# christang/alignment-algos

Hardware: AMD Instinct MI355X
Metric: GCUPS (DP cell updates/s) at 1/2/4/8 MI355X; bit-exact score vs ref (higher is better)
Workload: dtype int32

## Files before the change

### alignment-algos_amd/csrc/aln_device.h

```cpp
#pragma once
#include "aln_internal.h"

namespace aln {

__device__ __forceinline__ float clip0(float s, bool local) {
  return local ? ((0.f < s) ? s : 0.f) : s;
}
__device__ __forceinline__ float fminr(float a, float b) { return (b < a) ? b : a; }

struct EvalDev {
  int Q, T;
  int model, align_type;
  float gi, ge;
  const float* tgi;
  const float* tge;
  const float* tcn;
  const float* deltab;
  const int64_t* deltab_off;
  const float* instab;
  int sim_kind;
  const uint8_t* qc; const uint8_t* tc;
  const float* tablef;
  const float* S; int ld;
};

__device__ __forceinline__ float dev_deletion(const EvalDev& e, int t1, int t2) {
  const bool free_end = (e.align_type == ALN_LOCAL || e.align_type == ALN_SEMI_LOCAL || e.align_type == ALN_LOCAL_GLOBAL);
  if (e.model == ALN_GAP_AFFINE_CONST) {
    int len = t2 - t1 - 1;
    if (len < 1) return 0.f;
    if (free_end && (t1 == 0 || t2 == e.T - 1)) return 0.f;
    return e.gi + e.ge * (float)(len - 1);
  } else if (e.model == ALN_GAP_DEL_TABLE_INS_TPOS || e.model == ALN_GAP_TABLES) {
    return e.deltab[(size_t)t1 * e.T + t2];
  } else {
    int dist = t2 - t1;
    if (dist < 2) return 0.f;
    float gi = fminr(e.tgi[t1], e.tgi[t2]);
    float ge = fminr(e.tge[t1], e.tge[t2]);
    if (free_end && (t1 == 0 || t2 == e.T - 1)) return 0.f;
    return gi + ge * (float)(dist - 2);
  }
}
__device__ __forceinline__ float dev_insertion(const EvalDev& e, int q1, int q2, int t1, int t2) {
  const bool free_end = (e.align_type == ALN_LOCAL || e.align_type == ALN_SEMI_LOCAL || e.align_type == ALN_GLOBAL_LOCAL);
  if (e.model == ALN_GAP_AFFINE_CONST) {
    int len = q2 - q1 - 1;
    if (len < 1) return 0.f;
    if (free_end && (q1 == 0 || q2 == e.Q - 1)) return 0.f;
    return e.gi + e.ge * (float)(len - 1);
  } else if (e.model == ALN_GAP_TABLES) {
    const size_t QT = (size_t)e.Q * e.T;
    if (q1 == 0) return e.instab[QT + (size_t)t1 * e.Q + q2];
    if (q2 == e.Q - 1) return e.instab[2 * QT + (size_t)t1 * e.Q + q1];
    return e.instab[(size_t)t1 * e.Q + (q2 - q1)];
  } else if (e.model == ALN_GAP_DEL_TABLE_INS_TPOS) {
    int dist = q2 - q1;
    if (dist < 2) return 0.f;
    float gp = e.tgi[t1] + e.tge[t1] * (float)(dist - 2);
    gp = gp + e.tcn[t1];
    if (free_end && (q1 == 0 || q2 == e.Q - 1)) return 0.f;
    return gp;
  } else {
    int dist = q2 - q1;
    if (dist < 2) return 0.f;
    float gi = fminr(e.tgi[t1], e.tgi[t2]);
    float ge = fminr(e.tge[t1], e.tge[t2]);
    if (free_end && (q1 == 0 || q2 == e.Q - 1)) return 0.f;
    return gi + ge * (float)(dist - 2);
  }
}
__device__ __forceinline__ void bind_table_model(EvalDev& e, const EvalDev& proto, const PairDesc& pd) {
  e.tcn = proto.tcn ? proto.tcn + pd.t_off : nullptr;
  e.deltab = proto.deltab ? proto.deltab + proto.deltab_off[pd.t_seq] : nullptr;
  e.instab = proto.instab ? proto.instab + pd.ins_off : nullptr;
}
__device__ __forceinline__ float dev_sim(const EvalDev& e, int i, int j) {
  if (e.sim_kind == ALN_SIM_SUBMATRIX) {
    if (i <= 0 || j <= 0 || i >= e.Q - 1 || j >= e.T - 1) return 0.f;
    return e.tablef[(int)e.qc[i] * 32 + (int)e.tc[j]];
  }
  return e.S[(size_t)i * e.ld + j] + 0.0f;
}

struct Frame {
  int q0, q1, t0, t1, rev;
  __device__ __forceinline__ int nQ() const { return q1 - q0; }
  __device__ __forceinline__ int nT() const { return t1 - t0; }
  __device__ __forceinline__ int rq(int a) const { return rev ? q1 - a : q0 + a; }
  __device__ __forceinline__ int rt(int b) const { return rev ? t1 - b : t0 + b; }
};

__device__ __forceinline__ float frame_del(const EvalDev& e, const Frame& f, int blo, int bhi) {
  int x = f.rt(blo), y = f.rt(bhi);
  return dev_deletion(e, x < y ? x : y, x < y ? y : x);
}
__device__ __forceinline__ float frame_ins(const EvalDev& e, const Frame& f, int alo, int ahi, int blo, int bhi) {
  int x = f.rq(alo), y = f.rq(ahi), u = f.rt(blo), v = f.rt(bhi);
  return dev_insertion(e, x < y ? x : y, x < y ? y : x, u < v ? u : v, u < v ? v : u);
}

__device__ __forceinline__ uint32_t pack_ptr(int pq, int pt) { return ((uint32_t)pq << 16) | ((uint32_t)pt & 0xFFFFu); }

__host__ __device__ __forceinline__ void decode_ptr(uint32_t w, int mode, int i, int j, int& pq, int& pt) {
  if (w == 0xFFFFFFFFu) { pq = -1; pt = -1; return; }
  if (mode == 0) { pq = (int)(w >> 16); pt = (int)(w & 0xFFFFu); if (pq == 0xFFFF) pq = -1; if (pt == 0xFFFF) pt = -1; return; }
  const int tb = mode == 2 ? 12 : 11, tmax = (1 << tb) - 1;
  const int prio = (int)((w >> tb) & 3u), k = tmax - (int)(w & (uint32_t)tmax);
  if (prio == 3) { pq = i - 1; pt = j - 1; }
  else if (prio == 2) { pq = i - 1; pt = k; }
  else { pq = k; pt = j - 1; }
}
__host__ __device__ __forceinline__ uint32_t load_ptr_word(const uint32_t* Pbase, int64_t plane_off, int ld, int i, int j, int mode) {
  const size_t e = (size_t)plane_off + (size_t)i * ld + j;
  if (mode == 0) return Pbase[e];
  const uint16_t w = reinterpret_cast<const uint16_t*>(Pbase)[e];
  return w == 0xFFFFu ? 0xFFFFFFFFu : (uint32_t)w;
}
__host__ __device__ __forceinline__ void store_ptr_word(uint32_t* Pbase, int64_t plane_off, int ld, int i, int j, int mode, uint32_t w) {
  const size_t e = (size_t)plane_off + (size_t)i * ld + j;
  if (mode == 0) Pbase[e] = w;
  else reinterpret_cast<uint16_t*>(Pbase)[e] = (uint16_t)(w & 0xFFFFu);
}
__host__ __device__ __forceinline__ float load_score(const float* Hbase, int64_t plane_off, int ld, int i, int j, int hmode) {
  const size_t e = (size_t)plane_off + (size_t)i * ld + j;
  if (hmode == 0) return Hbase[e];
  return (float)reinterpret_cast<const uint16_t*>(Hbase)[e];
}
__host__ __device__ __forceinline__ float flag_score(uint32_t w) { return (w != 0xFFFFFFFFu && (w & 0x8000u)) ? 1.f : 0.f; }
__host__ __device__ __forceinline__ void store_score(float* Hbase, int64_t plane_off, int ld, int i, int j, int hmode, float v) {
  const size_t e = (size_t)plane_off + (size_t)i * ld + j;
  if (hmode == 0) Hbase[e] = v;
  else reinterpret_cast<uint16_t*>(Hbase)[e] = (uint16_t)(int)v;
}
__host__ __device__ __forceinline__ uint32_t encode_ptr(int mode, int i, int j, int pq, int pt) {
  if (mode == 0) return ((uint32_t)pq << 16) | ((uint32_t)pt & 0xFFFFu);
  const int tb = mode == 2 ? 12 : 11, tmax = (1 << tb) - 1;
  if (pq == i - 1 && pt == j - 1) return 3u << tb;
  if (pq == i - 1) return (2u << tb) | (uint32_t)(tmax - pt);
  return (1u << tb) | (uint32_t)(tmax - pq);
}

}
```

### alignment-algos_amd/csrc/dp_affine_tag.hip

```cpp
#include <algorithm>
#include <cmath>
#include <cstdio>
#include <cstdlib>

#include "aln_internal.h"
#include "dp_tag_common.h"

namespace aln {

__device__ __forceinline__ void setprio_dyn(int p) {
  switch (p & 3) {
    case 0: __builtin_amdgcn_s_setprio(0); break;
    case 1: __builtin_amdgcn_s_setprio(1); break;
    case 2: __builtin_amdgcn_s_setprio(2); break;
    default: __builtin_amdgcn_s_setprio(3); break;
  }
}

template <int NW, int R, bool LOCAL, bool H16, int KBT, int X, bool SEGQ, int TB, int OCC, bool LEAN = false>
__global__ __launch_bounds__(64 * NW) __attribute__((amdgpu_waves_per_eu(R * X == 16 ? OCC : 1, R * X == 16 ? OCC : 8))) void dp_affine_tag_kernel(
    const PairDesc* __restrict__ pairs, const uint8_t* __restrict__ qcodes, const uint8_t* __restrict__ tcodes,
    const int32_t* __restrict__ table32, float* __restrict__ Hbase, uint32_t* __restrict__ Pbase,
    PairResult* __restrict__ res, TagParams prm) {
  typedef TagBits<TB> tag;
  constexpr int TAGMAX = tag::TAGMAX, P_MATCH = tag::P_MATCH, P_DEL = tag::P_DEL, P_INS = tag::P_INS;
  constexpr int ZKEY = tag::ZKEY, ORIGIN_DEL = tag::ORIGIN_DEL, ORIGIN_INS = tag::ORIGIN_INS;
  constexpr int KB = (KBT == 16) ? 16 : TB + 2;
  constexpr int LOW = (1 << KB) - 1;
  constexpr int NEGK = (KBT == 16) ? -(1 << 29) : tag::NEGK;
  static_assert(KBT == 13 || (KBT == 16 && LOCAL && H16), "the 16-bit key layout needs non-negative 15-bit scores");
  static_assert(TB == 11 || TB == 12, "11 or 12 tag bits");
  static_assert(X == 4 || X == 8, "a lane owns 4 or 8 consecutive columns of each group");
  static_assert(!LEAN || (NW == 2 && R == 2 && X == 8 && LOCAL && H16 && KBT == 16 && TB == 11 && !SEGQ), "one lean shape: the 16-bit key layout, whole pairs");
  constexpr int GW = 64 * X;
  __shared__ int tab[32 * 32];
  __shared__ uint8_t qcs[1 << TB];
  constexpr int RING = 16;
  __shared__ __attribute__((aligned(16))) int xch[RING][NW][4];
  __shared__ int red[NW][2];

  __shared__ int s_item;
  int pair_id = blockIdx.x, seg = 0;
  if constexpr (SEGQ) {
    if (threadIdx.x == 0) {
      const int t = __hip_atomic_fetch_add(&prm.queue[0], 1, __ATOMIC_RELAXED, __HIP_MEMORY_SCOPE_AGENT) + 1;
      int item;
      if (t < prm.n_pairs) item = t * 8;
      else {
        const int* slot = &prm.queue[16 + (t - prm.n_pairs)];
        long spins = 0;
        while ((item = __hip_atomic_load(slot, __ATOMIC_RELAXED, __HIP_MEMORY_SCOPE_AGENT)) < 0) {
          __builtin_amdgcn_s_sleep(32);
          if (++spins > (1L << 24)) {
            __hip_atomic_store(&prm.queue[2], 1, __ATOMIC_RELAXED, __HIP_MEMORY_SCOPE_AGENT);
            item = -2;
            break;
          }
        }
        __builtin_amdgcn_fence(__ATOMIC_ACQUIRE, "agent");
        asm volatile("s_waitcnt vmcnt(0)" ::: "memory");
      }
      s_item = item;
    }
    __syncthreads();
    const int item = s_item;
    if (item < 0) return;
    pair_id = item >> 3; seg = item & 7;
  }
  const PairDesc pd = pairs[pair_id];
  const int Q = pd.Q, T = pd.T, ld = pd.ld;
  const int n_seg = SEGQ ? seg_count(Q, prm.ksegs) : 1;
  const int i_begin = seg_bound(Q, seg, n_seg), i_end = seg_bound(Q, seg + 1, n_seg);
  const int lane = threadIdx.x & 63;
  const int w = __builtin_amdgcn_readfirstlane(threadIdx.x >> 6);
  const int W0 = w * GW * R;
  const int cb = W0 + X * lane;
  const int gi = prm.gi, ge = prm.ge;
  float* __restrict__ H = Hbase + pd.plane_off;
  uint16_t* __restrict__ P = reinterpret_cast<uint16_t*>(Pbase) + pd.plane_off;
  const uint8_t* __restrict__ qc = qcodes + pd.q_off;
  const uint8_t* __restrict__ tc = tcodes + pd.t_off;

  for (int k = threadIdx.x; k < 32 * 32; k += 64 * NW) tab[k] = table32[k] * (1 << KB);
  for (int k = threadIdx.x; k < Q; k += 64 * NW) qcs[k] = qc[k];
  __syncthreads();

  int inm[R][X];
  int code4[R][X];
  int GK[R][X];
  int EK[R][X];
  bool inrange[R];
#pragma unroll
  for (int r = 0; r < R; ++r) {
    inrange[r] = (cb + GW * r) < ld;
#pragma unroll
    for (int x = 0; x < X; ++x) {
      const int c = cb + GW * r + x;
      int code = kCodeTail;
      if (c < T) code = tc[c];
      code4[r][x] = code * 4;
      inm[r][x] = ((unsigned)(c - 1) < (unsigned)(T - 2)) ? -1 : 0;
      GK[r][x] = (((ge * c) * (1 << KB)) | P_DEL | (TAGMAX - (c & TAGMAX))) - P_MATCH;
      EK[r][x] = (ge * c + gi - ge) * (1 << KB);
    }
  }
  const int CB = W0 + GW * R;
  int codeB4 = kCodeTail * 4;
  if (NW > 1 && CB < T) codeB4 = tc[CB] * 4;

  int dk[R][X];
  int gmx[R][X];
  int cvk[R];
  int ak[R][X];
  uint32_t pf[R][X];
#pragma unroll
  for (int r = 0; r < R; ++r) {
    cvk[r] = NEGK;
#pragma unroll
    for (int x = 0; x < X; ++x) { dk[r][x] = P_MATCH; gmx[r][x] = NEGK; pf[r][x] = kNullPtr; }
  }
  int lmax = P_MATCH; uint32_t lpos = 0;
  const int lag = (NW > 1) ? prm.lag : 0;

  typedef unsigned int u32x2 __attribute__((ext_vector_type(2)));
  typedef unsigned int u32x4 __attribute__((ext_vector_type(4)));
  uint16_t* const H16p = reinterpret_cast<uint16_t*>(Hbase) + pd.plane_off;
  const int vo16 = cb * 2;
  auto store_words = [&](const uint32_t (&wd)[X / 2], __amdgpu_buffer_rsrc_t rs, int off) {
    if constexpr (X == 4) { const u32x2 v = {wd[0], wd[1]}; __builtin_amdgcn_raw_buffer_store_b64(v, rs, off, 0, 0); }
    else { const u32x4 v = {wd[0], wd[1], wd[2], wd[3]}; __builtin_amdgcn_raw_buffer_store_b128(v, rs, off, 0, 0); }
  };
  int own_r = -1;
  uint32_t flag_bits = 0x80008000u, sel_high = 0x07060302u;
  if constexpr (LEAN) {
    asm volatile("" : "+v"(flag_bits), "+v"(sel_high));
    const int tchunk = (T - 2) / X;
    own_r = ((tchunk & 63) == lane) ? (tchunk >> 6) - w * R : -1;
  }
  auto store_row = [&](int i, bool border = false) {
    const size_t ro = (size_t)i * ld + cb;
    const __amdgpu_buffer_rsrc_t rsP = __builtin_amdgcn_make_buffer_rsrc(P + (size_t)i * ld, 0, ld * 2, 0x00020000);
    const __amdgpu_buffer_rsrc_t rsH = __builtin_amdgcn_make_buffer_rsrc(H16p + (size_t)i * ld, 0, ld * 2, 0x00020000);
    if constexpr (LEAN) {
      const bool whole = i == Q - 2;
      asm volatile("" : "+v"(own_r));
#pragma unroll
      for (int r = 0; r < R; ++r) {
        uint32_t pw[X / 2], hw[X / 2];
#pragma unroll
        for (int x = 0; x < X; x += 2) {
          pw[x / 2] = __builtin_amdgcn_perm(pf[r][x + 1], pf[r][x], 0x05040100u);
          hw[x / 2] = __builtin_amdgcn_perm((uint32_t)dk[r][x + 1], (uint32_t)dk[r][x], sel_high);
          pw[x / 2] |= (hw[x / 2] + 0x7FFF7FFFu) & flag_bits;
        }
        if (whole || (!border && own_r == r)) store_words(hw, rsH, vo16 + 2 * GW * r);
        store_words(pw, rsP, vo16 + 2 * GW * r);
      }
      return;
    }
#pragma unroll
    for (int r = 0; r < R; ++r) {
      uint32_t pw[X / 2], hw[X / 2];
#pragma unroll
      for (int x = 0; x < X; x += 2) pw[x / 2] = __builtin_amdgcn_perm(pf[r][x + 1], pf[r][x], 0x05040100u);
      if (H16) {
#pragma unroll
        for (int x = 0; x < X; x += 2)
          hw[x / 2] = (KBT == 16) ? __builtin_amdgcn_perm((uint32_t)dk[r][x + 1], (uint32_t)dk[r][x], 0x07060302u)
                                  : (((uint32_t)dk[r][x] >> KB) | (((uint32_t)dk[r][x + 1] >> KB) << 16));
        store_words(hw, rsH, vo16 + 2 * GW * r);
      } else if (inrange[r]) {
        const float sc = 1.0f / (float)(1 << KB);
#pragma unroll
        for (int x = 0; x < X; x += 4)
          *reinterpret_cast<float4*>(H + ro + GW * r + x) =
              make_float4((float)(dk[r][x] - P_MATCH) * sc, (float)(dk[r][x + 1] - P_MATCH) * sc, (float)(dk[r][x + 2] - P_MATCH) * sc,
                          (float)(dk[r][x + 3] - P_MATCH) * sc);
      }
      store_words(pw, rsP, vo16 + 2 * GW * r);
    }
  };
  auto tab_at = [&](int qrow, int c4) -> int {
    return *reinterpret_cast<const int*>(reinterpret_cast<const char*>(tab) + qrow + c4);
  };

  auto finish_row = [&](int i, int dB, uint32_t pB, bool sync, const int4 (&xin)[NW > 1 ? NW - 1 : 1]) {
    int sk = NEGK;
    int ik[R];
#pragma unroll
    for (int r = 0; r < R; ++r) {
#pragma unroll
      for (int x = 0; x < X; ++x) ak[r][x] = dk[r][x] + GK[r][x];
      int a0 = ak[r][0];
      if (r == 0) a0 = (lane == 0) ? NEGK : a0;
      int t0 = max(a0, ak[r][1]), t1 = max(ak[r][2], ak[r][3]);
      if constexpr (X == 8) { t0 = max(max(t0, ak[r][4]), ak[r][5]); t1 = max(max(t1, ak[r][6]), ak[r][7]); }
      ik[r] = max(t0, t1);
    }
    wave_incl_max_keys<R>(ik);
#pragma unroll
    for (int r = 0; r < R; ++r) {
      const int ek = tdpp<0x138>(NEGK, ik[r]);
      cvk[r] = max(sk, ek);
      sk = max(sk, __builtin_amdgcn_readlane(ik[r], 63));
    }
    if (NW > 1) {
      const int slot = i & (RING - 1);
      if (lane == 63) { xch[slot][w][0] = sk; xch[slot][w][1] = dB; xch[slot][w][2] = (int)pB; }
      if (sync) asm volatile("s_waitcnt lgkmcnt(0)\n\ts_barrier" ::: "memory");
      if (w > 0) {
        int fk = NEGK;
        int d0 = P_MATCH; uint32_t p0 = kNullPtr;
#pragma unroll
        for (int v = 0; v < NW - 1; ++v) {
          if (v < w) {
            const int4 t = sync ? *reinterpret_cast<const int4*>(&xch[slot][v][0]) : xin[v];
            fk = max(fk, t.x);
            if (v < w - 1) {
              const int Cn = (v + 1) * GW * R;
              fk = max(fk, t.y + ((((ge * Cn) * (1 << KB)) | P_DEL | (TAGMAX - Cn)) - P_MATCH));
            } else {
              d0 = t.y; p0 = (uint32_t)t.z;
            }
          }
        }
        if (lane == 0) { dk[0][0] = d0; pf[0][0] = p0; ak[0][0] = d0 + GK[0][0]; }
        const int f2 = max(fk, d0 + ((((ge * W0) * (1 << KB)) | P_DEL | (TAGMAX - W0)) - P_MATCH));
#pragma unroll
        for (int r = 0; r < R; ++r) {
          int nv = max(f2, cvk[r]);
          if (r == 0) nv = (lane == 0) ? fk : nv;
          cvk[r] = nv;
        }
      }
    }
    if (LOCAL) {
      int rm = P_MATCH;
#pragma unroll
      for (int r = 0; r < R; ++r)
#pragma unroll
        for (int x = 0; x < X; x += 2) rm = max(max(rm, dk[r][x]), dk[r][x + 1]);
      if (rm > lmax) {
        lmax = rm;
        int cfirst = 0x7FFFFFFF;
#pragma unroll
        for (int r = R - 1; r >= 0; --r)
#pragma unroll
          for (int x = X - 1; x >= 0; --x) cfirst = (dk[r][x] == rm) ? (cb + GW * r + x) : cfirst;
        lpos = ((uint32_t)i << 16) | (uint32_t)cfirst;
      }
    }
    store_row(i);
  };

  constexpr int kStateChunks = (2 * R * X + R + 2 + 3) / 4;
  constexpr int kStateBytes = kStateChunks * 16 * 64 * NW;
  auto state_rsrc = [&](int pr, int sgm) {
    char* base = *reinterpret_cast<char* volatile*>(&prm.queue[4]);
    return __builtin_amdgcn_make_buffer_rsrc(base + ((size_t)pr * kSegs + sgm) * kStateBytes, 0, kStateBytes, 0x00020000);
  };
  auto state_words = [&](uint32_t (&wv)[kStateChunks * 4], bool save) {
    int n = 0;
#pragma unroll
    for (int r = 0; r < R; ++r)
#pragma unroll
      for (int x = 0; x < X; ++x) { if (save) wv[n] = (uint32_t)dk[r][x]; else dk[r][x] = (int)wv[n]; ++n; }
#pragma unroll
    for (int r = 0; r < R; ++r)
#pragma unroll
      for (int x = 0; x < X; ++x) { if (save) wv[n] = (uint32_t)gmx[r][x]; else gmx[r][x] = (int)wv[n]; ++n; }
#pragma unroll
    for (int r = 0; r < R; ++r) { if (save) wv[n] = (uint32_t)cvk[r]; else cvk[r] = (int)wv[n]; ++n; }
    if (save) { wv[n] = (uint32_t)lmax; wv[n + 1] = lpos; } else { lmax = (int)wv[n]; lpos = wv[n + 1]; }
  };

  if (SEGQ && seg > 0) {
    const __amdgpu_buffer_rsrc_t rs = state_rsrc(pair_id, seg - 1);
    uint32_t wv[kStateChunks * 4] = {};
#pragma unroll
    for (int c = 0; c < kStateChunks; ++c) {
      const u32x4 v = __builtin_amdgcn_raw_buffer_load_b128(rs, (c * 64 * NW + (int)threadIdx.x) * 16, 0, 16);
      wv[4 * c] = v.x; wv[4 * c + 1] = v.y; wv[4 * c + 2] = v.z; wv[4 * c + 3] = v.w;
    }
    state_words(wv, false);
#pragma unroll
    for (int r = 0; r < R; ++r)
#pragma unroll
      for (int x = 0; x < X; ++x) ak[r][x] = dk[r][x] + GK[r][x];
  }
  if (seg == 0) store_row(0, true);
  if (seg == 0 && Q >= 3) {
    const int qrow = (int)qcs[1] * 128;
    auto row1 = [&](int c, int sK, int& dkv, uint32_t& pv) {
      const int cost = (c >= 2 && !prm.free_del) ? ((gi + ge * (c - 2)) * (1 << KB)) : 0;
      int v = sK - cost;
      if (LOCAL) v = max(v, 0);
      const bool in = (unsigned)(c - 1) < (unsigned)(T - 2);
      dkv = (in ? v : 0) | P_MATCH;
      pv = in ? (uint32_t)(c == 1 ? P_MATCH : ORIGIN_DEL) : kNullPtr;
    };
#pragma unroll
    for (int r = 0; r < R; ++r)
#pragma unroll
      for (int x = 0; x < X; ++x) row1(cb + GW * r + x, tab_at(qrow, code4[r][x]), dk[r][x], pf[r][x]);
    int dB = P_MATCH; uint32_t pB = kNullPtr;
    if (NW > 1) row1(CB, tab_at(qrow, codeB4), dB, pB);
    const int4 none[NW > 1 ? NW - 1 : 1] = {};
    finish_row(1, dB, pB, true, none);
  }

  const int lane_row4 = (lane & 31) * 4;
  const int hwslot = (int)__builtin_amdgcn_s_getreg((3 << 11) | (0 << 6) | 4);
  int code_n1 = (int)qcs[min(i_begin + 1, Q - 1)];
  int rowv_next = tab_at((int)qcs[min(i_begin, Q - 1)] * 128, lane_row4);
  const int it_end = i_end - 1 + lag * (NW - 1);
  for (int it = i_begin; it <= it_end; ++it) {
    const int i = it - lag * w;
    const bool sync = lag == 0;
    if (i >= i_begin && i < i_end) {
    int4 xin[NW > 1 ? NW - 1 : 1];
    if (NW > 1 && !sync && w > 0) {
#pragma unroll
      for (int v = 0; v < NW - 1; ++v) if (v < w) xin[v] = *reinterpret_cast<const int4*>(&xch[i & (RING - 1)][v][0]);
    }
    const int par = (i ^ hwslot) & 1;
    if (prm.alt_prio & 0x100) {
      setprio_dyn(par ? (prm.alt_prio >> 4) & 3 : prm.alt_prio & 3);
    } else if (prm.alt_prio == 1) {
      if (par) __builtin_amdgcn_s_setprio(3); else __builtin_amdgcn_s_setprio(0);
    } else if (prm.alt_prio == 2) {
      __builtin_amdgcn_s_setprio(0);
    } else if (prm.alt_prio == 3) {
      if (par) __builtin_amdgcn_s_setprio(1); else __builtin_amdgcn_s_setprio(0);
    }
    const int rowv = rowv_next;
    rowv_next = tab_at(code_n1 * 128, lane_row4);
    code_n1 = (int)qcs[min(i + 2, Q - 1)];
    const int FK = (gi + ge * (i - 2)) * (1 << KB);
    const int RK = (((ge * (i - 1)) * (1 << KB)) | P_INS | (TAGMAX - (i - 1))) - P_MATCH;
    const int colK = prm.free_ins ? 0 : FK;

    int bk[R][X];
    int sv[R][X];
#pragma unroll
    for (int r = 0; r < R; ++r)
#pragma unroll
      for (int x = 0; x < X; ++x) sv[r][x] = __builtin_amdgcn_ds_bpermute(code4[r][x], rowv);
    const int svB = (NW > 1) ? __builtin_amdgcn_ds_bpermute(codeB4, rowv) : 0;
#pragma unroll
    for (int r = 0; r < R; ++r) {
      int pv = cvk[r];
#pragma unroll
      for (int x = 0; x < X; ++x) {
        const int m = dk[r][x];
        int A = ak[r][x];
        if (r == 0 && x == 0) A = (cb == 0) ? NEGK : A;
        const int e = pv - EK[r][x];
        const int f = gmx[r][x] - FK;
        bk[r][x] = max(max(m, e), f);
        pv = max(pv, A);
      }
    }
    int dB = P_MATCH; uint32_t pB = kNullPtr;
    if (NW > 1) {
      int kh = bk[R - 1][X - 1] + svB;
      if (LOCAL) kh = max(kh, ZKEY);
      const bool in = CB <= T - 2;
      dB = in ? ((kh & ~LOW) | P_MATCH) : P_MATCH;
      pB = in ? (uint32_t)(kh & LOW) : kNullPtr;
    }
#pragma unroll
    for (int r = 0; r < R; ++r)
#pragma unroll
      for (int x = 0; x < X; ++x) {
        gmx[r][x] = max(gmx[r][x], dk[r][x] + RK);
        asm volatile("" : "+v"(gmx[r][x]));
      }
    int prev_k = 0;
#pragma unroll
    for (int r = 0; r < R; ++r) {
      const int uk = (r == 0) ? __builtin_amdgcn_update_dpp(0, bk[r][X - 1], 0x138, 0xF, 0xF, true) : tdpp<0x138>(prev_k, bk[r][X - 1]);
      prev_k = __builtin_amdgcn_readlane(bk[r][X - 1], 63);
      const bool masked = (r == 0 && W0 == 0) || (W0 + GW * (r + 1) > T - 1);
      int sK1 = 0;
#pragma unroll
      for (int x = 0; x < X; ++x) {
        const int sK = sv[r][x];
        if (r == 0 && x == 1) sK1 = sK;
        int kh = ((x == 0) ? uk : bk[r][x - 1]) + sK;
        if (LOCAL) kh = max(kh, ZKEY);
        dk[r][x] = (kh & ~LOW) | P_MATCH;
        pf[r][x] = (KBT == 16) ? (uint32_t)kh : (uint32_t)(kh & LOW);
      }
      if (masked) {
        asm volatile("" ::: "memory");
        if (r == 0) {
          int v1 = sK1 - colK;
          if (LOCAL) v1 = max(v1, 0);
          const bool is1 = cb == 0;
          dk[0][1] = is1 ? (v1 | P_MATCH) : dk[0][1]; pf[0][1] = is1 ? (uint32_t)ORIGIN_INS : pf[0][1];
        }
#pragma unroll
        for (int x = 0; x < X; ++x) {
          dk[r][x] = (dk[r][x] & inm[r][x]) | P_MATCH;
          pf[r][x] |= ~(uint32_t)inm[r][x];
        }
      }
    }
    if (prm.alt_prio & 0x100) setprio_dyn(par ? (prm.alt_prio >> 6) & 3 : (prm.alt_prio >> 2) & 3);
    else if (prm.alt_prio == 2) __builtin_amdgcn_s_setprio(3);
    else if (prm.alt_prio == 3) { if (par) __builtin_amdgcn_s_setprio(3); else __builtin_amdgcn_s_setprio(2); }
    finish_row(i, dB, pB, sync, xin);
    }
    if (NW > 1 && !sync && (it & (lag - 1)) == lag - 1) asm volatile("s_waitcnt lgkmcnt(0)\n\ts_barrier" ::: "memory");
  }

  int pair_out = pair_id;
  if constexpr (SEGQ) {
    const int item = *reinterpret_cast<volatile int*>(&s_item);
    pair_out = item >> 3;
    const int seg_out = item & 7;
    if (seg_out + 1 < seg_count(Q, prm.ksegs)) {
    const __amdgpu_buffer_rsrc_t rs = state_rsrc(pair_out, seg_out);
    uint32_t wv[kStateChunks * 4] = {};
    state_words(wv, true);
#pragma unroll
    for (int c = 0; c < kStateChunks; ++c) {
      const u32x4 v = {wv[4 * c], wv[4 * c + 1], wv[4 * c + 2], wv[4 * c + 3]};
      __builtin_amdgcn_raw_buffer_store_b128(v, rs, (c * 64 * NW + (int)threadIdx.x) * 16, 0, 16);
    }
    asm volatile("s_waitcnt vmcnt(0)" ::: "memory");
    __syncthreads();
    if (threadIdx.x == 0) {
      const int idx = __hip_atomic_fetch_add(&prm.queue[1], 1, __ATOMIC_RELAXED, __HIP_MEMORY_SCOPE_AGENT) + 1;
      __hip_atomic_store(&prm.queue[16 + idx], item + 1, __ATOMIC_RELAXED, __HIP_MEMORY_SCOPE_AGENT);
    }
    return;
    }
  }

  if (Q >= 2) {
#pragma unroll
    for (int r = 0; r < R; ++r)
#pragma unroll
      for (int x = 0; x < X; ++x) { dk[r][x] = P_MATCH; pf[r][x] = kNullPtr; }
    store_row(Q - 1, true);
  }

  if (LOCAL) {
    int m = lmax;
#pragma unroll
    for (int o = 32; o >= 1; o >>= 1) m = max(m, __shfl_xor(m, o));
    uint32_t p = (lmax == m && (m >> KB) > 0) ? lpos : 0xFFFFFFFFu;
#pragma unroll
    for (int o = 32; o >= 1; o >>= 1) p = min(p, (uint32_t)__shfl_xor((int)p, o));
    if (NW > 1) {
      if (lane == 0) { red[w][0] = m; red[w][1] = (int)p; }
      __syncthreads();
      int gm = 0;
      for (int v = 0; v < NW; ++v) gm = max(gm, red[v][0]);
      uint32_t gp = 0xFFFFFFFFu;
      for (int v = 0; v < NW; ++v) if (red[v][0] == gm) gp = min(gp, (uint32_t)red[v][1]);
      m = gm; p = gp;
    }
    if (threadIdx.x == 0) { res[pair_out].part_max = (float)(m >> KB); res[pair_out].part_pos = p; }
  } else {
    if (threadIdx.x == 0) { res[pair_out].part_max = 0.f; res[pair_out].part_pos = 0xFFFFFFFFu; }
  }
}


int tag_path_bits(const aln_batch* b, const float* table, int n, const aln_gap* gap) {
  if (!table || gap->model != ALN_GAP_AFFINE_CONST) return 0;
  if (b->maxQ > 4096 || b->maxT > 4096) return 0;
  const float gi = gap->gap_init, ge = gap->gap_extn;
  if (!(gi == (float)(int)gi) || !(ge == (float)(int)ge) || gi < 0 || ge < 0) return 0;
  double maxs = 0;
  for (int k = 0; k < n * n; ++k) {
    const float v = table[k];
    if (!(v == (float)(int)v)) return 0;
    if (fabs((double)v) > maxs) maxs = fabs((double)v);
  }
  const double mn = (double)std::min(b->maxQ, b->maxT), mx = (double)std::max(b->maxQ, b->maxT);
  if (b->maxQ <= 2048 && b->maxT <= 2048 && b->ctx->hints.tag_bits != 12)
    return (maxs + ge) * ((double)b->maxQ + (double)b->maxT) + gi + maxs < 65536.0 ? 11 : 0;
  return (maxs * mn + 2 * gi + 3 * ge * mx + maxs < 100000.0 && gi + ge * mx < 16000.0) ? 12 : 0;
}
bool tag_path_legal(const aln_batch* b, const float* table, int n, const aln_gap* gap) { return tag_path_bits(b, table, n, gap) != 0; }
bool tag_h16_legal(const aln_batch* b) {
  double maxs = 0;
  for (float v : b->h_table) maxs = std::max(maxs, fabs((double)v));
  return maxs * (double)std::min(b->maxQ, b->maxT) < 65536.0;
}

bool tag_key16_legal(const aln_batch* b) {
  double maxs = 0;
  for (float v : b->h_table) maxs = std::max(maxs, fabs((double)v));
  const double gi = b->gap.gap_init, ge = b->gap.gap_extn;
  const double L = (double)std::max(b->maxQ, b->maxT), best = maxs * (double)std::min(b->maxQ, b->maxT);
  return best + ge * L + maxs < 32767.0 && gi + ge * L + maxs < 8000.0;
}

template <int NW, int R, int X, int TB>
static int launch_tag_variant(aln_batch* b, const TagParams& prm_in) {
  TagParams prm = prm_in;
  while (prm.lag * NW > 16) prm.lag >>= 1;
  dim3 grid(b->n_pairs), block(64 * NW);
  hipStream_t st = b->ctx->stream;
  const int want = b->ctx->hints.tag_segments;
  prm.n_pairs = b->n_pairs; prm.queue = nullptr;
  prm.ksegs = std::min(std::abs(want), kSegs);
  bool segq = false;
  if (prm.ksegs >= 1 && (want < 0 || (b->n_pairs >= 512 && R * X == 16))) {
    long items = 0;
    for (const PairDesc& d : b->h_pairs) items += seg_count(d.Q, prm.ksegs);
    if (items > b->n_pairs || prm.ksegs == 1) {
      constexpr size_t kStateBytes = (size_t)((2 * R * X + R + 2 + 3) / 4) * 16 * 64 * NW;
      const size_t qbytes = ((size_t)(16 + std::max<long>(items - b->n_pairs, 4)) * 4 + 15) & ~(size_t)15;
      const size_t sbytes = (size_t)b->n_pairs * kSegs * kStateBytes;
      if (b->tagq_bytes < qbytes || b->tagstate_bytes < sbytes) {
        ALN_HIP_CHECK(b->ctx, hipStreamSynchronize(st));
        hipFree(b->d_tagq); hipFree(b->d_tagstate); b->d_tagq = nullptr; b->d_tagstate = nullptr; b->tagq_bytes = b->tagstate_bytes = 0;
        ALN_HIP_CHECK(b->ctx, hipMalloc((void**)&b->d_tagq, qbytes));
        ALN_HIP_CHECK(b->ctx, hipMalloc((void**)&b->d_tagstate, sbytes));
        b->tagq_bytes = qbytes; b->tagstate_bytes = sbytes;
        ALN_HIP_CHECK(b->ctx, hipMemcpy(b->d_tagq + 4, &b->d_tagstate, 8, hipMemcpyHostToDevice));
      }
      ALN_HIP_CHECK(b->ctx, hipMemsetAsync(b->d_tagq, 0xFF, 16, st));
      ALN_HIP_CHECK(b->ctx, hipMemsetAsync(b->d_tagq + 16, 0xFF, qbytes - 64, st));
      prm.queue = b->d_tagq;
      grid = dim3((unsigned)items);
      segq = true;
    }
  }
  b->tag_segmented = segq;
  const bool k16 = b->islocal && b->h_mode == 1 && tag_key16_legal(b) && b->ctx->hints.key16;
  const int occ_hint = b->ctx->hints.tag_occupancy;
  const long wps = ((long)b->n_pairs * NW + 1023) / 1024;
  const bool auto3 = ((wps + 2) / 3) * 45 < ((wps + 1) / 2) * 32;
  const bool occ3 = R * X == 16 && !segq && (occ_hint == 3 || (occ_hint == 0 && auto3));
  constexpr bool kLeanShape = NW == 2 && R == 2 && X == 8 && TB == 11;
  const bool lean = kLeanShape && b->lean_request && k16 && !segq;
#define ALN_TAG_LAUNCH_O(LOC_, H16_, KB_, SQ_, OCC_)                                                                                 \
  hipLaunchKernelGGL((dp_affine_tag_kernel<NW, R, LOC_, H16_, KB_, X, SQ_, TB, OCC_>), grid, block, 0, st, b->d_pairs, b->d_qcodes, b->d_tcodes, \
                     b->d_table32, b->d_H, b->d_P, b->d_res, prm)
#define ALN_TAG_LAUNCH(LOC_, H16_, KB_, SQ_) do {                                                                                    \
    if constexpr (R * X == 16 && !(SQ_)) { if (occ3) ALN_TAG_LAUNCH_O(LOC_, H16_, KB_, SQ_, 3); else ALN_TAG_LAUNCH_O(LOC_, H16_, KB_, SQ_, 2); } \
    else ALN_TAG_LAUNCH_O(LOC_, H16_, KB_, SQ_, 2);                                                                                  \
  } while (0)
#define ALN_TAG_LAUNCH_Q(LOC_, H16_, KB_) do { if (segq) ALN_TAG_LAUNCH(LOC_, H16_, KB_, true); else ALN_TAG_LAUNCH(LOC_, H16_, KB_, false); } while (0)
  if constexpr (kLeanShape) {
    if (lean) {
      if (occ3) hipLaunchKernelGGL((dp_affine_tag_kernel<NW, R, true, true, 16, X, false, TB, 3, true>), grid, block, 0, st, b->d_pairs, b->d_qcodes,
                                   b->d_tcodes, b->d_table32, b->d_H, b->d_P, b->d_res, prm);
      else hipLaunchKernelGGL((dp_affine_tag_kernel<NW, R, true, true, 16, X, false, TB, 2, true>), grid, block, 0, st, b->d_pairs, b->d_qcodes,
                              b->d_tcodes, b->d_table32, b->d_H, b->d_P, b->d_res, prm);
    }
  }
  if (lean) {}
  else if (k16) ALN_TAG_LAUNCH_Q(true, true, 16);
  else if (b->islocal && b->h_mode == 1) ALN_TAG_LAUNCH_Q(true, true, 13);
  else if (b->islocal) ALN_TAG_LAUNCH_Q(true, false, 13);
  else ALN_TAG_LAUNCH_Q(false, false, 13);
#undef ALN_TAG_LAUNCH_Q
#undef ALN_TAG_LAUNCH
#undef ALN_TAG_LAUNCH_O
  char nm[96];
  snprintf(nm, sizeof nm, "dp_affine_tag_kernel<NW=%d,R=%d,%s%s%s%s%s%s%s>%s", NW, R, X == 8 ? "X=8," : "", b->islocal ? "local" : "global",
           b->h_mode == 1 ? ",h16" : "", k16 ? ",key16" : "", TB == 12 ? ",tag12" : "", lean ? ",lean" : "", occ3 ? ",occ3" : "", segq ? "+segq" : "");
  b->kernel_name = nm;
  b->planes_lean = lean;
  ALN_HIP_CHECK(b->ctx, hipGetLastError());
  return ALN_OK;
}

int launch_dp_affine_tag(aln_batch* b) {
  TagParams prm;
  prm.gi = (int)b->gap.gap_init;
  prm.ge = (int)b->gap.gap_extn;
  prm.free_del = b->gapdev.free_del;
  prm.free_ins = b->gapdev.free_ins;
  prm.alt_prio = b->ctx->hints.tag_alt_prio;
  prm.lag = b->ctx->hints.tag_lag;
  if (prm.lag < 0 || prm.lag > 4 || (prm.lag & (prm.lag - 1))) prm.lag = 0;
  const int ld = b->maxld;
  int nw = b->ctx->hints.dp_nw, r = b->ctx->hints.dp_r, x = b->ctx->hints.dp_x ? b->ctx->hints.dp_x : 4;
  if (b->ptr_mode == 2) return launch_tag_variant<4, 2, 8, 12>(b, prm);
  if (nw == 0) {
    if (ld <= 256) { nw = 1; r = 1; }
    else if (ld <= 512) { nw = 2; r = 1; }
    else if (ld <= 1024) { nw = 4; r = 1; }
    else { nw = 2; r = 2; x = 8; }
  }
  if (64 * x * nw * r < ld) return ALN_E_TOO_LONG;
#define ALN_V(NW_, R_, X_) if (nw == NW_ && r == R_ && x == X_) return launch_tag_variant<NW_, R_, X_, 11>(b, prm)
  ALN_V(1, 1, 4); ALN_V(1, 2, 4); ALN_V(1, 4, 4); ALN_V(1, 8, 4);
  ALN_V(2, 1, 4); ALN_V(2, 2, 4); ALN_V(2, 4, 4);
  ALN_V(4, 1, 4); ALN_V(4, 2, 4);
  ALN_V(8, 1, 4);
  ALN_V(1, 4, 8); ALN_V(2, 1, 8); ALN_V(2, 2, 8); ALN_V(4, 1, 8);
#undef ALN_V
  return ALN_E_ARG;
}

}
```

### alignment-algos_amd/csrc/traceback.hip

```cpp
#include "aln_device.h"

namespace aln {

struct TbParams {
  int islocal;
  int subali;
  int rev;
  int stride;
  int ptr_mode;
  int h_mode;
};

__global__ __launch_bounds__(64) void traceback_kernel(const PairDesc* __restrict__ pairs, const float* __restrict__ Hbase,
                                                       const uint32_t* __restrict__ Pbase, PairResult* __restrict__ res,
                                                       int32_t* __restrict__ out, TbParams prm) {
  const PairDesc pd = pairs[blockIdx.x];
  const int ld = pd.ld, lane = threadIdx.x;
  int32_t* o = out + (size_t)blockIdx.x * prm.stride * 2;
  PairResult r = res[blockIdx.x];
  if (r.status == ALN_E_HIP) return;
  const int Q = pd.Q, T = pd.T;
  const int sg = prm.rev ? 1 : -1;
  int n = 0, status = 0;
  auto emit1 = [&](int q, int t) {
    if (n < prm.stride) { if (lane == 0) { o[2 * n] = q; o[2 * n + 1] = t; } }
    else status = ALN_E_OVERFLOW;
    ++n;
  };
  int q, t, qstop, tstop;
  if (prm.subali) { q = pd.q1; t = pd.t1; qstop = pd.q0; tstop = pd.t0; }
  else if (prm.rev) { q = 0; t = 0; qstop = Q - 1; tstop = T - 1; }
  else { q = Q - 1; t = T - 1; qstop = 0; tstop = 0; }
  emit1(q, t);
  if (prm.islocal && !prm.subali) { q = r.best_q; t = r.best_t; emit1(q, t); }
  int lq = q, lt = t;
  auto before_stop = [&](int x) { return prm.rev ? (x < qstop) : (x > qstop); };
  while (before_stop(q)) {
    const int cq = q + sg * lane, ct = t + sg * lane;
    const bool valid = cq >= 0 && ct >= 0 && cq < Q && ct < T;
    uint32_t p = kNullPtr; float h = 0.f;
    if (valid) {
      p = load_ptr_word(Pbase, pd.plane_off, ld, cq, ct, prm.ptr_mode);
      h = prm.h_mode == 2 ? flag_score(p) : load_score(Hbase, pd.plane_off, ld, cq, ct, prm.h_mode);
    }
    const float hnext = __shfl_down(h, 1);
    const bool active = valid && before_stop(cq);
    const int nq_ = cq + sg, nt_ = ct + sg;
    int dq_, dt_;
    decode_ptr(p, prm.ptr_mode, cq, ct, dq_, dt_);
    const bool diag = active && p != kNullPtr && nq_ >= 0 && nt_ >= 0 && nq_ < Q && nt_ < T && dq_ == nq_ && dt_ == nt_;
    bool go = diag && lane < 63;
    if (prm.islocal) go = go && !(hnext <= 0.f);
    const unsigned long long m = __ballot(go);
    const int L = (~m == 0ull) ? 64 : __builtin_ctzll(~m);
    if (lane < L) {
      int k = n + lane;
      if (k < prm.stride) { o[2 * k] = nq_; o[2 * k + 1] = nt_; }
    }
    if (n + L > prm.stride) status = ALN_E_OVERFLOW;
    n += L;
    const int sq = q + sg * L, st = t + sg * L;
    const uint32_t pL = (uint32_t)__shfl((int)p, L);
    const int jq = __shfl(dq_, L), jt = __shfl(dt_, L);
    const bool diagL = __shfl((int)diag, L) != 0;
    q = sq; t = st; lq = sq; lt = st;
    if (!before_stop(sq)) break;
    if (diagL && L == 63) continue;
    if (diagL) { lq = sq + sg; lt = st + sg; break; }
    const int nq = jq, nt = jt;
    if (pL == kNullPtr) { lq = -1; lt = -1; if (!prm.islocal) status = ALN_E_STARTPAIR; break; }
    if (prm.islocal) {
      const float hn = prm.h_mode == 2 ? flag_score(load_ptr_word(Pbase, pd.plane_off, ld, nq, nt, prm.ptr_mode))
                                       : load_score(Hbase, pd.plane_off, ld, nq, nt, prm.h_mode);
      if (hn <= 0.f) { lq = nq; lt = nt; break; }
    }
    emit1(nq, nt);
    q = nq; t = nt; lq = nq; lt = nt;
  }
  if (prm.islocal && !prm.subali) {
    if (lq != qstop && lt != tstop) emit1(qstop, tstop);
  } else {
    if (lq != qstop || lt != tstop) status = ALN_E_STARTPAIR;
  }
  if (lane == 0) {
    r.n_path = n < prm.stride ? n : prm.stride;
    r.status = status;
    res[blockIdx.x] = r;
  }
}

int launch_traceback(aln_batch* b, bool subali) {
  TbParams prm;
  prm.islocal = (b->islocal && !subali) ? 1 : 0;
  prm.subali = subali ? 1 : 0;
  prm.rev = (b->direction == ALN_REV && !subali) ? 1 : 0;
  prm.stride = b->path_stride;
  prm.ptr_mode = b->ptr_mode;
  prm.h_mode = b->planes_lean ? 2 : b->h_mode;
  hipLaunchKernelGGL(traceback_kernel, dim3(b->n_pairs), dim3(64), 0, b->ctx->stream, b->d_pairs, b->d_H, b->d_P,
                     b->d_res, b->d_path, prm);
  ALN_HIP_CHECK(b->ctx, hipGetLastError());
  if (!subali) { b->optimal_build = b->n_builds; b->optimal_since_build = true; }
  return ALN_OK;
}

}
```

Baseline: 1754.

## Encode lean-mode zero-score flag via clipped key instead of per-cell H bit

In the lean plane mode, the per-cell perm/add/and that packed a positive-score flag into the pointer word is removed. Zero-clipped local cells are now recognised because the clip key carries a low bit (CLIPK = ZKEY|1), which produces a distinct pointer pattern that traceback decodes as zero, with explicit zero bits set only at the boundary cells. The H perm is now computed only for rows that actually store H. Lean mode also forces the wavefront lag to zero and simplifies the priority switching. This trims inner-loop ALU work in the store path, at the cost of a subtler encoding that must stay bit-exact with the reference.

```diff
diff --git a/alignment-algos_amd/csrc/aln_device.h b/alignment-algos_amd/csrc/aln_device.h
--- a/alignment-algos_amd/csrc/aln_device.h
+++ b/alignment-algos_amd/csrc/aln_device.h
@@ -127,7 +127,11 @@
   if (hmode == 0) return Hbase[e];
   return (float)reinterpret_cast<const uint16_t*>(Hbase)[e];
 }
-__host__ __device__ __forceinline__ float flag_score(uint32_t w) { return (w != 0xFFFFFFFFu && (w & 0x8000u)) ? 1.f : 0.f; }
+constexpr uint32_t kLeanZeroBit = 0x8000u;
+constexpr uint32_t kLeanZeroMatch = (3u << 11) | 1u;
+__host__ __device__ __forceinline__ float lean_score(uint32_t w) {
+  return (w == 0xFFFFFFFFu || w == kLeanZeroMatch || (w & kLeanZeroBit)) ? 0.f : 1.f;
+}
 __host__ __device__ __forceinline__ void store_score(float* Hbase, int64_t plane_off, int ld, int i, int j, int hmode, float v) {
   const size_t e = (size_t)plane_off + (size_t)i * ld + j;
   if (hmode == 0) Hbase[e] = v;
diff --git a/alignment-algos_amd/csrc/dp_affine_tag.hip b/alignment-algos_amd/csrc/dp_affine_tag.hip
--- a/alignment-algos_amd/csrc/dp_affine_tag.hip
+++ b/alignment-algos_amd/csrc/dp_affine_tag.hip
@@ -3,6 +3,7 @@
 #include <cstdio>
 #include <cstdlib>
 
+#include "aln_device.h"
 #include "aln_internal.h"
 #include "dp_tag_common.h"
 
@@ -28,6 +29,8 @@
   constexpr int KB = (KBT == 16) ? 16 : TB + 2;
   constexpr int LOW = (1 << KB) - 1;
   constexpr int NEGK = (KBT == 16) ? -(1 << 29) : tag::NEGK;
+  constexpr int CLIPK = LEAN ? (ZKEY | 1) : ZKEY;
+  constexpr uint32_t ZBIT = LEAN ? kLeanZeroBit : 0u;
   static_assert(KBT == 13 || (KBT == 16 && LOCAL && H16), "the 16-bit key layout needs non-negative 15-bit scores");
   static_assert(TB == 11 || TB == 12, "11 or 12 tag bits");
   static_assert(X == 4 || X == 8, "a lane owns 4 or 8 consecutive columns of each group");
@@ -120,7 +123,7 @@
     for (int x = 0; x < X; ++x) { dk[r][x] = P_MATCH; gmx[r][x] = NEGK; pf[r][x] = kNullPtr; }
   }
   int lmax = P_MATCH; uint32_t lpos = 0;
-  const int lag = (NW > 1) ? prm.lag : 0;
+  const int lag = (NW > 1 && !LEAN) ? prm.lag : 0;
 
   typedef unsigned int u32x2 __attribute__((ext_vector_type(2)));
   typedef unsigned int u32x4 __attribute__((ext_vector_type(4)));
@@ -130,30 +133,31 @@
     if constexpr (X == 4) { const u32x2 v = {wd[0], wd[1]}; __builtin_amdgcn_raw_buffer_store_b64(v, rs, off, 0, 0); }
     else { const u32x4 v = {wd[0], wd[1], wd[2], wd[3]}; __builtin_amdgcn_raw_buffer_store_b128(v, rs, off, 0, 0); }
   };
+  int whole_row = Q - 2;
   int own_r = -1;
-  uint32_t flag_bits = 0x80008000u, sel_high = 0x07060302u;
   if constexpr (LEAN) {
-    asm volatile("" : "+v"(flag_bits), "+v"(sel_high));
     const int tchunk = (T - 2) / X;
     own_r = ((tchunk & 63) == lane) ? (tchunk >> 6) - w * R : -1;
+    asm volatile("" : "+s"(whole_row));
   }
   auto store_row = [&](int i, bool border = false) {
     const size_t ro = (size_t)i * ld + cb;
     const __amdgpu_buffer_rsrc_t rsP = __builtin_amdgcn_make_buffer_rsrc(P + (size_t)i * ld, 0, ld * 2, 0x00020000);
     const __amdgpu_buffer_rsrc_t rsH = __builtin_amdgcn_make_buffer_rsrc(H16p + (size_t)i * ld, 0, ld * 2, 0x00020000);
     if constexpr (LEAN) {
-      const bool whole = i == Q - 2;
+      const bool whole = i == whole_row;
       asm volatile("" : "+v"(own_r));
 #pragma unroll
       for (int r = 0; r < R; ++r) {
-        uint32_t pw[X / 2], hw[X / 2];
-#pragma unroll
-        for (int x = 0; x < X; x += 2) {
-          pw[x / 2] = __builtin_amdgcn_perm(pf[r][x + 1], pf[r][x], 0x05040100u);
-          hw[x / 2] = __builtin_amdgcn_perm((uint32_t)dk[r][x + 1], (uint32_t)dk[r][x], sel_high);
-          pw[x / 2] |= (hw[x / 2] + 0x7FFF7FFFu) & flag_bits;
+        uint32_t pw[X / 2];
+#pragma unroll
+        for (int x = 0; x < X; x += 2) pw[x / 2] = __builtin_amdgcn_perm(pf[r][x + 1], pf[r][x], 0x05040100u);
+        if (whole || (!border && own_r == r)) {
+          uint32_t hw[X / 2];
+#pragma unroll
+          for (int x = 0; x < X; x += 2) hw[x / 2] = __builtin_amdgcn_perm((uint32_t)dk[r][x + 1], (uint32_t)dk[r][x], 0x07060302u);
+          store_words(hw, rsH, vo16 + 2 * GW * r);
         }
-        if (whole || (!border && own_r == r)) store_words(hw, rsH, vo16 + 2 * GW * r);
         store_words(pw, rsP, vo16 + 2 * GW * r);
       }
       return;
@@ -297,7 +301,7 @@
       if (LOCAL) v = max(v, 0);
       const bool in = (unsigned)(c - 1) < (unsigned)(T - 2);
       dkv = (in ? v : 0) | P_MATCH;
-      pv = in ? (uint32_t)(c == 1 ? P_MATCH : ORIGIN_DEL) : kNullPtr;
+      pv = in ? (uint32_t)(c == 1 ? P_MATCH : ORIGIN_DEL) | (v == 0 ? ZBIT : 0u) : kNullPtr;
     };
 #pragma unroll
     for (int r = 0; r < R; ++r)
@@ -324,7 +328,9 @@
       for (int v = 0; v < NW - 1; ++v) if (v < w) xin[v] = *reinterpret_cast<const int4*>(&xch[i & (RING - 1)][v][0]);
     }
     const int par = (i ^ hwslot) & 1;
-    if (prm.alt_prio & 0x100) {
+    if constexpr (LEAN) {
+      if (prm.alt_prio == 1) { if (par) __builtin_amdgcn_s_setprio(3); else __builtin_amdgcn_s_setprio(0); }
+    } else if (prm.alt_prio & 0x100) {
       setprio_dyn(par ? (prm.alt_prio >> 4) & 3 : prm.alt_prio & 3);
     } else if (prm.alt_prio == 1) {
       if (par) __builtin_amdgcn_s_setprio(3); else __builtin_amdgcn_s_setprio(0);
@@ -364,7 +370,7 @@
     int dB = P_MATCH; uint32_t pB = kNullPtr;
     if (NW > 1) {
       int kh = bk[R - 1][X - 1] + svB;
-      if (LOCAL) kh = max(kh, ZKEY);
+      if (LOCAL) kh = max(kh, CLIPK);
       const bool in = CB <= T - 2;
       dB = in ? ((kh & ~LOW) | P_MATCH) : P_MATCH;
       pB = in ? (uint32_t)(kh & LOW) : kNullPtr;
@@ -388,7 +394,7 @@
         const int sK = sv[r][x];
         if (r == 0 && x == 1) sK1 = sK;
         int kh = ((x == 0) ? uk : bk[r][x - 1]) + sK;
-        if (LOCAL) kh = max(kh, ZKEY);
+        if (LOCAL) kh = max(kh, CLIPK);
         dk[r][x] = (kh & ~LOW) | P_MATCH;
         pf[r][x] = (KBT == 16) ? (uint32_t)kh : (uint32_t)(kh & LOW);
       }
@@ -398,7 +404,7 @@
           int v1 = sK1 - colK;
           if (LOCAL) v1 = max(v1, 0);
           const bool is1 = cb == 0;
-          dk[0][1] = is1 ? (v1 | P_MATCH) : dk[0][1]; pf[0][1] = is1 ? (uint32_t)ORIGIN_INS : pf[0][1];
+          dk[0][1] = is1 ? (v1 | P_MATCH) : dk[0][1]; pf[0][1] = is1 ? ((uint32_t)ORIGIN_INS | (v1 == 0 ? ZBIT : 0u)) : pf[0][1];
         }
 #pragma unroll
         for (int x = 0; x < X; ++x) {
@@ -407,7 +413,8 @@
         }
       }
     }
-    if (prm.alt_prio & 0x100) setprio_dyn(par ? (prm.alt_prio >> 6) & 3 : (prm.alt_prio >> 2) & 3);
+    if constexpr (LEAN) {}
+    else if (prm.alt_prio & 0x100) setprio_dyn(par ? (prm.alt_prio >> 6) & 3 : (prm.alt_prio >> 2) & 3);
     else if (prm.alt_prio == 2) __builtin_amdgcn_s_setprio(3);
     else if (prm.alt_prio == 3) { if (par) __builtin_amdgcn_s_setprio(3); else __builtin_amdgcn_s_setprio(2); }
     finish_row(i, dB, pB, sync, xin);
diff --git a/alignment-algos_amd/csrc/traceback.hip b/alignment-algos_amd/csrc/traceback.hip
--- a/alignment-algos_amd/csrc/traceback.hip
+++ b/alignment-algos_amd/csrc/traceback.hip
@@ -41,7 +41,7 @@
     uint32_t p = kNullPtr; float h = 0.f;
     if (valid) {
       p = load_ptr_word(Pbase, pd.plane_off, ld, cq, ct, prm.ptr_mode);
-      h = prm.h_mode == 2 ? flag_score(p) : load_score(Hbase, pd.plane_off, ld, cq, ct, prm.h_mode);
+      h = prm.h_mode == 2 ? lean_score(p) : load_score(Hbase, pd.plane_off, ld, cq, ct, prm.h_mode);
     }
     const float hnext = __shfl_down(h, 1);
     const bool active = valid && before_stop(cq);
@@ -70,7 +70,7 @@
     const int nq = jq, nt = jt;
     if (pL == kNullPtr) { lq = -1; lt = -1; if (!prm.islocal) status = ALN_E_STARTPAIR; break; }
     if (prm.islocal) {
-      const float hn = prm.h_mode == 2 ? flag_score(load_ptr_word(Pbase, pd.plane_off, ld, nq, nt, prm.ptr_mode))
+      const float hn = prm.h_mode == 2 ? lean_score(load_ptr_word(Pbase, pd.plane_off, ld, nq, nt, prm.ptr_mode))
                                        : load_score(Hbase, pd.plane_off, ld, nq, nt, prm.h_mode);
       if (hn <= 0.f) { lq = nq; lt = nt; break; }
     }
```

Measured after the change: 1924 (median of 6 runs). 1.1x the previous value.
